# cvxgrp/qcqp

Hardware: AMD Instinct MI355X
Metric: restarts x coord-sweeps / sec (improve COORD_DESCENT phase-2 sweeps, 2n^2 flops each; whole step timed) (higher is better)
Workload: dtype f64

## Files before the change

qcqp_amd/csrc/capi.hip:

```cpp
#include <dlfcn.h>
#include <unistd.h>
#include <hip/hip_runtime.h>
#include <rccl/rccl.h>

#include <algorithm>
#include <cmath>
#include <cstdarg>
#include <cstdio>
#include <cstring>
#include <string>
#include <chrono>
#include <vector>

#include "../../include/qcqp_mi.h"
#include "kernels.hip"
#include "admm.h"
#include "admm_fused.h"
#include "cd_queue.h"
#include "cd_life.h"
#include "gemm_pk.h"
#include "cd_general.h"
#include "cd_dense.h"
#include "sdr_solve.h"

// ... 129 lines not shown
    double stream_limit = 16e9;
    double *dn_gp_pre = nullptr, *dn_tmp = nullptr;
    ncclComm_t comm = nullptr;
    int rank = 0, world = 1;
    double *d_comm = nullptr, *d_comm_big = nullptr;
    int64_t comm_big_cap = 0;
    long long *d_prof = nullptr;
    int cd_stage = 0;
    int64_t Xi_cap = 0;
    bool sdr_factor_resident = false;
    double ad_Minv_rho = 0.0;
    bool ad_Minv_device = false;
    const char *last_cd2_kernel = "";
    bool profile = false;
    int dbg = 0;
    char *af_work = nullptr;
    size_t af_work_cap = 0;
    bool ad_fused = true;
    int ad_fused_nt = 512;
    const char *last_admm_kernel = "";
    int last_admm_C = 0;
    long long af_prof[16] = {0};
    int cd_queue = 2;
    int *d_qnext = nullptr;
    bool q_prepared = false;
    CdLife *d_life = nullptr;
    int Kreal = 0;
    double fbound = 0.0;
    double *l2_scratch = nullptr; size_t l2_scratch_cap = 0;
    double *l2_D = nullptr, *l2_S = nullptr;
    int *l2_abort = nullptr;
    int *l2_cuslot = nullptr;
    double *l2_preslack = nullptr; int64_t l2_preslack_cap = 0;
    double *lr_L = nullptr, *lr_G = nullptr, *lr_U = nullptr; int lr_RB = 0;
    int life_version = 0;
    long long *d_life_prof = nullptr;
    int64_t *d_bestK_idx = nullptr; double *d_bestK_key = nullptr, *d_bestK_x = nullptr; int64_t bestK_cap = 0;
    bool cd_ref_order = false;
    bool force_generic = false;
    std::vector<int> last_st1, last_st2;
};

namespace {

void admm_free(qcqpmi_ctx *c, bool keep_zsolver);

int fail(qcqpmi_ctx *c, int code, const char *fmt, ...) {
    char buf[1024];
    va_list ap;
    va_start(ap, fmt);
    vsnprintf(buf, sizeof(buf), fmt, ap);
    va_end(ap);
    if (c) c->err = buf; else g_create_error = buf;
    return code;
}

#define HIPCHK(c, expr)                                                                       \
    do {                                                                                      \
        hipError_t e_ = (expr);                                                               \
        if (e_ != hipSuccess)                                                                 \
            return fail(c, QCQPMI_EHIP, "%s failed: %s (%s:%d)", #expr, hipGetErrorString(e_), \
                        __FILE__, __LINE__);                                                  \
    } while (0)

template <typename T>
int dev_alloc(qcqpmi_ctx *c, T **p, size_t count, bool zero = true) {
// ... 452 lines not shown
    if (!out || n <= 0 || m < 0) return fail(nullptr, QCQPMI_EINVAL, "ctx_create: bad arguments");
    int ndev = qcqpmi_device_count();
    if (ndev <= 0)
        return fail(nullptr, QCQPMI_EHIP, "no HIP device visible: the qcqp_amd engine requires an MI355X (there is no CPU fallback)");
    if (device < 0 || device >= ndev) return fail(nullptr, QCQPMI_EINVAL, "device %d out of range (%d visible)", device, ndev);
    qcqpmi_ctx *c = new qcqpmi_ctx();
    c->device = device; c->n = n; c->m = m; c->n16 = (n + 15) / 16 * 16;
    c->quads.resize((size_t)m + 1);
    if (const char *sl = getenv("QCQPMI_STREAM_LIMIT")) { const double v = atof(sl); if (v > 0.0) c->stream_limit = v; }
    hipError_t e = hipSetDevice(device);
    if (e == hipSuccess) e = hipStreamCreateWithFlags(&c->stream, hipStreamNonBlocking);
    for (int i = 0; i < 5 && e == hipSuccess; i++) {
        e = hipEventCreate(&c->timers[i].beg);
        if (e == hipSuccess) e = hipEventCreate(&c->timers[i].end);
    }
    if (e != hipSuccess) {
        int rc = fail(nullptr, QCQPMI_EHIP, "ctx_create: %s", hipGetErrorString(e));
        delete c;
        return rc;
    }
    *out = c;
    return 0;
}

void qcqpmi_ctx_destroy(qcqpmi_ctx *c) {
    if (!c) return;
    (void)hipSetDevice(c->device);
    if (c->stream) (void)spin_sync(c->stream);
    if (c->comm && rccl() && rccl()->CommDestroy) rccl()->CommDestroy(c->comm);
    free_population(c);
    admm_free(c, false);
    for (void *p : c->prob_allocs) (void)hipFree(p);
    void *ptrs[] = {c->d_Fpack, c->d_Frow, c->d_mu, c->d_best_idx, c->d_best_key, c->d_comm, c->d_comm_big,
                    c->dn_G, c->dn_Dg, c->dn_Ft, c->dn_prof, c->dn_state, c->d_planes, c->d_out, c->d_wS, c->d_wY, c->d_ww, c->d_wz, c->af_work, c->d_qnext, c->d_life, c->d_life_prof, c->d_bestK_idx, c->d_bestK_key, c->d_bestK_x, c->l2_scratch, c->l2_D, c->l2_S, c->l2_abort, c->l2_cuslot, c->l2_preslack, c->lr_L, c->lr_G, c->lr_U};
    if (c->h_out) (void)hipHostFree(c->h_out);
    if (c->h_pin) (void)hipHostFree(c->h_pin);
    for (void *p : ptrs) if (p) (void)hipFree(p);
    for (auto &t : c->timers) { if (t.beg) (void)hipEventDestroy(t.beg); if (t.end) (void)hipEventDestroy(t.end); }
    for (auto &e : c->dn_ev) if (e) (void)hipEventDestroy(e);
    for (auto &e : c->dn_evn) if (e) (void)hipEventDestroy(e);
    if (c->dn_hn) (void)hipHostFree(c->dn_hn);
    if (c->stream2) (void)hipStreamDestroy(c->stream2);
    if (c->stream) (void)hipStreamDestroy(c->stream);
    delete c;
}

int qcqpmi_set_quad(qcqpmi_ctx *c, int64_t k, int format, const double *vals, const int64_t *idx,
                    const int64_t *ptr, int64_t nnz, const double *q, double r, int relop) {
    if (!c) return QCQPMI_EINVAL;
    if (c->finalized) return fail(c, QCQPMI_ESTATE, "set_quad after finalize");
    if (k < 0 || k > c->m || !q) return fail(c, QCQPMI_EINVAL, "set_quad: bad k or q");
    if ((k == 0) != (relop == 0) || relop < 0 || relop > 2)
        return fail(c, QCQPMI_EINVAL, "set_quad: relop %d invalid for function %lld", relop, (long long)k);
    HostQuad &h = c->quads[(size_t)k];
    h = HostQuad();
    const int64_t n = c->n;
    if (format == QCQPMI_FMT_DENSE) {
        if (!vals) return fail(c, QCQPMI_EINVAL, "set_quad: dense vals missing");
        for (int64_t i = 0; i < n; i++)
            for (int64_t j = 0; j < n; j++) {
                double v = vals[i * n + j];
                if (v != 0.0) { h.ci.push_back((int)i); h.cj.push_back((int)j); h.cv.push_back(v); }
            }
    } else if (format == QCQPMI_FMT_CSR) {
        if (!ptr || (nnz > 0 && (!idx || !vals))) return fail(c, QCQPMI_EINVAL, "set_quad: CSR arrays missing");
        for (int64_t i = 0; i < n; i++)
            for (int64_t e = ptr[i]; e < ptr[i + 1]; e++) {
// ... 737 lines not shown
    const bool lr = use2 && factor_rb > 0 && nmw == 3 && (kind == L2_KIND_BAND || kind == L2_KIND_GEN);
    if (lr) cs2 = 0;
    if (!use2) {
        if (!eligible || c->life_version != 1)
            return fail(c, QCQPMI_EUNSUPPORTED, "cd_stream_run: the lifecycle kernel needs separable constraints -- at most four classes of coordinates, at most two constraints "
                        "per coordinate --, a diagonal of P0 that is positive everywhere or zero everywhere, and 48 <= n <= 2304: use qcqpmi_cd_run per population");
        const int NBq = (int)(c->n16 / 16);
        cs = (c->dbg & 128) ? ((c->dbg >> 8) & 7) : 4;
        cs = cs > RQ_CSMAX ? RQ_CSMAX : cs;
        if (cs >= NBq) cs = 0;
        cs &= ~1;
        if (NBq - cs > RQ_NSIMD * RQ_MAXU || NBq < 3) return fail(c, QCQPMI_EUNSUPPORTED, "cd_stream_run: n = %lld outside the range of cd_phase2_qs_kernel (n <= 1024, at least 3 blocks of 16)", (long long)c->n);
    }
    if (generate && (rc = pop_reserve(c, K * R))) return rc;
    if (!c->d_qnext && (rc = dev_alloc(c, &c->d_qnext, 16))) return rc;
    if (!c->d_life) HIPCHK(c, hipMalloc((void **)&c->d_life, sizeof(CdLife)));
    HIPCHK(c, hipMemsetAsync(c->d_qnext, 0, 16 * sizeof(int), c->stream));
    CdLife L;
    L.on = 1; L.generate = generate ? 1 : 0; L.phase1 = phase1 ? 1 : 0; L.Rtotal = K * R; L.Rpop = R;
    L.seed = seed; L.seed_stride = seed_stride; L.first_index = first_index; L.first_stride = first_stride; L.viol_tol = viol_tol;
    L.sweeps1 = c->d_sweeps1; L.status1 = c->d_status1; L.ran2 = c->d_flag;
    L.prof = nullptr;
    const char *pre_ev = getenv("QCQPMI_L2_PREBUILT");
    const bool pre = lr && !(pre_ev && atoi(pre_ev) == 0);
    L.prebuilt = pre ? 1 : 0; L.preslack = nullptr;
    if (pre) {
        if (K * R > c->l2_preslack_cap) {
            if (c->l2_preslack) { HIPCHK(c, spin_sync(c->stream)); (void)hipFree(c->l2_preslack); c->l2_preslack = nullptr; c->l2_preslack_cap = 0; }
            if ((rc = dev_alloc(c, &c->l2_preslack, (size_t)(K * R)))) return rc;
            c->l2_preslack_cap = K * R;
        }
        L.preslack = c->l2_preslack;
    }
    if (c->profile) {
        if (!c->d_life_prof) HIPCHK(c, hipMalloc((void **)&c->d_life_prof, 24 * sizeof(long long)));
        HIPCHK(c, hipMemsetAsync(c->d_life_prof, 0, 24 * sizeof(long long), c->stream));
        L.prof = c->d_life_prof;
    }
    HIPCHK(c, hipMemcpyAsync(c->d_life, &L, sizeof(L), hipMemcpyHostToDevice, c->stream));
    HIPCHK(c, spin_sync(c->stream));
    int cus = 0;
    HIPCHK(c, hipDeviceGetAttribute(&cus, hipDeviceAttributeMultiprocessorCount, c->device));
    stm[1] = stnow();
    if (use2) {
        if ((rc = cd_life2_reserve(c, nmw, cus))) return rc;
        if (!lr && (c->dbg & 128)) { const int k2 = (c->dbg >> 8) & 7; if (nmw == 3 && (k2 == 0 || k2 == 2 || k2 == 4) && k2 < (int)(c->n16 / 16)) cs2 = k2; }
        const int tiles = cd_life2_tiles(c->dp, nmw, cs2, K * R, cus, 0, lr ? 1 : 0);
        int64_t wgs = (K * R + 16 * tiles - 1) / (16 * tiles);
        const int maxw = cd_life2_max_wgs(nmw, cus, tiles);
        if (wgs > maxw) wgs = maxw;
        if (c->dbg & 1024) { const int lim = (c->dbg >> 12) & 1023; if (lim > 0 && wgs > lim) wgs = lim; }
        CdLife2Args qa;
        qa.P = c->dp; qa.num_iters = num_iters; qa.tol = tol; qa.life = c->d_life;
        cd_queue_fill_batch(c, qa.b, seed, first_index);
        qa.b.R = K * R;
        qa.scratch = c->l2_scratch; qa.Dpack = c->l2_D; qa.Spack = c->l2_S; qa.abort = c->l2_abort; qa.fbound = c->fbound;
        { const char *ev = getenv("QCQPMI_L2_ROT"); const int rot = ev ? atoi(ev) : (lr ? 2 : 0); qa.cuslot = rot ? c->l2_cuslot : nullptr; qa.rotmode = rot; }
        if (qa.cuslot) HIPCHK(c, hipMemsetAsync(c->l2_cuslot, 0, 4096 * sizeof(int), c->stream));
        qa.dbg = (c->dbg & 2048) ? 1 : 0;
        qa.Gpack = lr ? c->lr_G : nullptr; qa.Upack = lr ? c->lr_U : nullptr; qa.RB = lr ? c->lr_RB : 0;
        qa.nclass = c->Kreal;
        const double l0 = stnow();
        (void)hipEventRecord(c->timers[2].beg, c->stream);
        const double l1 = stnow();
        hipError_t qe = pre ? (hipError_t)cd_life2_prep_launch(c->dp, c->d_life, c->X, K * R, num_iters, tol, c->stream) : hipSuccess;
        if (qe == hipSuccess) qe = (hipError_t)cd_life2_launch(qa, nmw, cs2, kind, tiles, (int)wgs, c->stream);
        const double l2 = stnow();
        (void)hipEventRecord(c->timers[2].end, c->stream);
        c->timers[2].valid = true;
        if (qe != hipSuccess) return fail(c, QCQPMI_EHIP, "cd_stream_run: %s", hipGetErrorString(qe));
        c->last_cd2_kernel = cd_life2_name(nmw, kind, tiles, lr ? 1 : 0);
        int ab = 0;
        HIPCHK(c, spin_sync(c->stream));
        const double l3 = stnow();
        HIPCHK(c, hipMemcpyAsync(&ab, c->l2_abort, sizeof(int), hipMemcpyDeviceToHost, c->stream));
        const double l4 = stnow();
        HIPCHK(c, spin_sync(c->stream));
        if (stt) fprintf(stderr, "cd_stream_run launch (ms): reserve %.3f, event %.3f, launch call %.3f, event + spin wait %.3f, copy call %.3f, sync %.3f\n", l0 - stm[1], l1 - l0, l2 - l1, l3 - l2, l4 - l3, stnow() - l4);
        if (ab) {
            HIPCHK(c, hipMemsetAsync(c->l2_abort, 0, sizeof(int), c->stream));
            c->R = 0;
            return fail(c, QCQPMI_EHIP, "cd_stream_run: a wait inside cd_life_kernel ran into its watchdog (internal error; no results)");
        }
    } else {
        CdQueueArgs qa;
        qa.P = c->dp; qa.num_iters = num_iters; qa.tol = tol;
        qa.life = c->d_life; qa.life_on = 1;
        cd_queue_fill_batch(c, qa.b, seed, first_index);
        qa.b.R = K * R;
        (void)hipEventRecord(c->timers[2].beg, c->stream);
        hipError_t qe = (hipError_t)cd_queue_launch(qa, cs, cus, c->stream);
        (void)hipEventRecord(c->timers[2].end, c->stream);
        c->timers[2].valid = true;
        if (qe != hipSuccess) return fail(c, QCQPMI_EHIP, "cd_stream_run: %s", hipGetErrorString(qe));
        HIPCHK(c, spin_sync(c->stream));
        c->last_cd2_kernel = "cd_phase2_qs_kernel<lifecycle>";
    }
    c->cd_stage = 0;
// ... 318 lines not shown
```

qcqp_amd/csrc/capi_admm.inc:

```

namespace {

struct RocblasApi {
    void *h = nullptr;
    int (*create)(void **) = nullptr;
    int (*destroy)(void *) = nullptr;
    int (*set_stream)(void *, hipStream_t) = nullptr;
};

RocblasApi *rocblas() {
    static RocblasApi api;
    static bool tried = false;
    if (!tried) {
        tried = true;
        const char *names[] = {"librocblas.so", "librocblas.so.5", "/opt/rocm/lib/librocblas.so"};
        for (const char *nm : names) {
            api.h = dlopen(nm, RTLD_NOW | RTLD_GLOBAL);
            if (api.h) break;
        }
        if (api.h) {
            api.create = (decltype(api.create))dlsym(api.h, "rocblas_create_handle");
            api.destroy = (decltype(api.destroy))dlsym(api.h, "rocblas_destroy_handle");
            api.set_stream = (decltype(api.set_stream))dlsym(api.h, "rocblas_set_stream");
        }
// ... 464 lines not shown
    const int64_t idx = (int64_t)blockIdx.x * blockDim.x + threadIdx.x;
    if (idx >= n16 * n16) return;
    const int64_t t = idx / (n16 * 16), rem = idx % (n16 * 16), i = rem / 16, j = 16 * t + (rem & 15);
    Xtm[idx] = (i == j) ? alpha : 0.0;
}

__global__ void zs_pack_sym_kernel(const double *__restrict__ Xtm, double *__restrict__ Apk, int64_t n16) {
    const int64_t idx = (int64_t)blockIdx.x * blockDim.x + threadIdx.x;
    if (idx >= n16 * n16) return;
    const int l = (int)(idx & 63);
    const int64_t fk = idx >> 6, KS = n16 / 4, rb = fk / KS, kk = fk % KS;
    Apk[idx] = Xtm[rb * n16 * 16 + (4 * kk + (l >> 4)) * 16 + (l & 15)];
}

__global__ void zs_update_kernel(double *__restrict__ Xtm, const double *__restrict__ Utm, const double *__restrict__ Ttm,
                                 int64_t n16, unsigned long long *__restrict__ resid_bits) {
    const int64_t idx = (int64_t)blockIdx.x * blockDim.x + threadIdx.x;
    double r = 0.0;
    if (idx < n16 * n16) {
        const int64_t t = idx / (n16 * 16), rem = idx % (n16 * 16), i = rem / 16, j = 16 * t + (rem & 15);
        Xtm[idx] = 2.0 * Xtm[idx] - Utm[idx];
        r = fabs(Ttm[idx] - (i == j ? 1.0 : 0.0));
    }
    __shared__ double red[256];
    red[threadIdx.x] = r;
    __syncthreads();
    for (int s = 128; s > 0; s >>= 1) {
        if ((int)threadIdx.x < s) red[threadIdx.x] = fmax(red[threadIdx.x], red[threadIdx.x + s]);
        __syncthreads();
    }
    if (threadIdx.x == 0) atomicMax(resid_bits, (unsigned long long)__double_as_longlong(red[0]));
}

int qcqpmi_admm_zsolver_device(qcqpmi_ctx *c, double rho, int64_t max_iter, double *resid_out, int64_t *iters_out) {
    if (!c) return QCQPMI_EINVAL;
    if (!c->finalized) return fail(c, QCQPMI_ESTATE, "admm_zsolver_device: context not finalized");
    HIPCHK(c, hipSetDevice(c->device));
    const int64_t n = c->n, n16 = c->n16, m = c->m, tot = n16 * n16;
    const int KBn = (int)(n16 / 16), nt = KBn;
    if (max_iter <= 0) max_iter = 80;
    hipStream_t st = c->stream;
    int rc;
    DevBuf<double> Mtm, Mpk, Xtm, Xpk, Ttm, Utm, rs;
    DevBuf<unsigned long long> rb;
    if ((rc = dev_alloc(c, &Mtm.p, (size_t)tot, false)) || (rc = dev_alloc(c, &Mpk.p, (size_t)tot, false)) ||
        (rc = dev_alloc(c, &Xtm.p, (size_t)tot, false)) || (rc = dev_alloc(c, &Xpk.p, (size_t)tot, false)) ||
        (rc = dev_alloc(c, &Ttm.p, (size_t)tot, false)) || (rc = dev_alloc(c, &Utm.p, (size_t)tot, false)) ||
        (rc = dev_alloc(c, &rs.p, (size_t)n16, false)) || (rc = dev_alloc(c, &rb.p, 1, false)))
        return rc;
    const dim3 gb((unsigned)((tot + 255) / 256)), tb(256);
    hipLaunchKernelGGL(zs_build_kernel, gb, tb, 0, st, c->dp.P0, n, n16, rho * (double)m, Mtm.p);
    hipLaunchKernelGGL(zs_pack_sym_kernel, gb, tb, 0, st, (const double *)Mtm.p, Mpk.p, n16);
    hipLaunchKernelGGL(zs_rowsum_kernel, dim3((unsigned)((n16 + 255) / 256)), tb, 0, st, (const double *)Mtm.p, n16, rs.p);
    HIPCHK(c, hipGetLastError());
    std::vector<double> hrs((size_t)n16);
    HIPCHK(c, hipMemcpyAsync(hrs.data(), rs.p, (size_t)n16 * sizeof(double), hipMemcpyDeviceToHost, st));
    HIPCHK(c, spin_sync(st));
    double nrm = 0.0;
    for (double v : hrs) nrm = std::max(nrm, v);
    if (!(nrm > 0.0) || !std::isfinite(nrm)) return fail(c, QCQPMI_EINVAL, "admm_zsolver_device: 2 (P0 + rho m I) is zero or not finite");
    hipLaunchKernelGGL(zs_scaled_identity_kernel, gb, tb, 0, st, Xtm.p, n16, 1.0 / nrm);
    double resid = INFINITY, prev = INFINITY;
    int64_t it = 0;
    for (; it < max_iter; it++) {
        hipLaunchKernelGGL(zs_pack_sym_kernel, gb, tb, 0, st, (const double *)Xtm.p, Xpk.p, n16);
        if ((rc = gemm_pk(c, Mpk.p, Xtm.p, Ttm.p, nullptr, KBn, KBn, nt, 1))) return rc;
        if ((rc = gemm_pk(c, Xpk.p, Ttm.p, Utm.p, nullptr, KBn, KBn, nt, 1))) return rc;
        HIPCHK(c, hipMemsetAsync(rb.p, 0, sizeof(unsigned long long), st));
        hipLaunchKernelGGL(zs_update_kernel, gb, tb, 0, st, Xtm.p, (const double *)Utm.p, (const double *)Ttm.p, n16, rb.p);
        HIPCHK(c, hipGetLastError());
        unsigned long long bits = 0;
        HIPCHK(c, hipMemcpyAsync(&bits, rb.p, sizeof bits, hipMemcpyDeviceToHost, st));
        HIPCHK(c, spin_sync(st));
        double r;
        memcpy(&r, &bits, sizeof r);
        prev = resid; resid = r;
        if (!std::isfinite(resid)) return fail(c, QCQPMI_EREFERENCE, "admm_zsolver_device: iteration diverged (is P0 + rho m I positive definite?)");
        if (resid < 1e-7 && (resid * resid < 1e-15 || resid >= 0.5 * prev)) { it++; break; }
        if (it > 8 && resid > 1.0 - 1e-12 && prev > 1.0 - 1e-12 && resid >= prev)
            return fail(c, QCQPMI_EREFERENCE, "admm_zsolver_device: no contraction (is P0 + rho m I positive definite?)");
    }
    if (!(resid < 1e-7)) return fail(c, QCQPMI_EREFERENCE, "admm_zsolver_device: not converged after %lld iterations (residual %.3e)", (long long)it, resid);
    if (c->ad_Minvpk) { (void)hipFree(c->ad_Minvpk); c->ad_Minvpk = nullptr; }
    if ((rc = dev_alloc(c, &c->ad_Minvpk, (size_t)tot, false))) return rc;
    hipLaunchKernelGGL(zs_pack_sym_kernel, gb, tb, 0, st, (const double *)Xtm.p, c->ad_Minvpk, n16);
    HIPCHK(c, hipGetLastError());
    HIPCHK(c, spin_sync(st));
    c->ad_Minv_rho = rho;
    c->ad_Minv_device = true;
    if (resid_out) *resid_out = resid * resid;
    if (iters_out) *iters_out = it;
    return 0;
}

__global__ __launch_bounds__(256) void p0_gemv_kernel(const double *__restrict__ P0, const double *__restrict__ v, int64_t n, int64_t n16,
                                                      double *__restrict__ y) {
    const int lane = threadIdx.x & 63;
    const int64_t row = (int64_t)blockIdx.x * 4 + (threadIdx.x >> 6);
    if (row >= n) return;
    const double *pr = P0 + row * n16;
    double s = 0.0;
    for (int64_t j = lane; j < n; j += 64) s += pr[j] * v[j];
    for (int off = 32; off > 0; off >>= 1) s += __shfl_down(s, off, 64);
    if (lane == 0) y[row] = s;
}

static double tridiag_min_eig(const std::vector<double> &al, const std::vector<double> &be, int k) {
    double lo = INFINITY, hi = -INFINITY;
    for (int i = 0; i < k; i++) {
        const double r = (i > 0 ? fabs(be[i - 1]) : 0.0) + (i + 1 < k ? fabs(be[i]) : 0.0);
        lo = std::min(lo, al[i] - r); hi = std::max(hi, al[i] + r);
    }
    auto count_below = [&](double x) {
        int cnt = 0; double d = 1.0;
        for (int i = 0; i < k; i++) {
// ... 466 lines not shown
```

qcqp_amd/csrc/cd_life.h:

```cpp
#pragma once
#include <hip/hip_runtime.h>
#include <stdint.h>
#include "kernels.h"
#include "cd_queue.h"

namespace qcqpmi {

enum { L2_KIND_BAND = 0, L2_KIND_GEN = 1, L2_KIND_LIN = 2, L2_KIND_GENK = 3, L2_KIND_LINK = 4 };

struct CdLife2Args {
    DevProblem P;
    CdBatch b;
    int64_t num_iters;
    double tol;
    const CdLife *life;
    double *scratch;
    const double *Dpack;
    const double *Spack;
    int *abort;
    int *cuslot;
    double fbound;
    const double *Gpack, *Upack;
    int RB;
    int rotmode;
    int nclass;
    int dbg;
};

bool cd_life2_config(const DevProblem &P, int Kreal, int objclass, bool symcls, int factor_rb, int *nmw, int *cs, int *kind);
size_t cd_life2_lds_bytes(int nmw, int cs, int tiles, int lr, int kind);
bool cd_life2_factor_ok(const DevProblem &P, int64_t r);
int cd_life2_pack_factor(const double *Lrow, double *Gpack, double *Upack, int NB, int RB, hipStream_t st);
int cd_life2_max_wgs(int nmw, int cus, int tiles);
int cd_life2_tiles(const DevProblem &P, int nmw, int cs, int64_t restarts, int cus, int requested, int lr);
int cd_life2_pack(const DevProblem &P, double *Dpack, double *Spack, hipStream_t st);
int cd_life2_prep_launch(const DevProblem &P, const CdLife *life, double *X, int64_t Rtotal, int64_t num_iters, double tol, hipStream_t st);
int cd_life2_launch(const CdLife2Args &a, int nmw, int cs, int kind, int tiles, int wgs, hipStream_t st);
const char *cd_life2_name(int nmw, int kind, int tiles, int lr);

}
```

qcqp_amd/csrc/cd_life.hip:

```cpp
#include "cd_life.h"

#include <cstdio>
#include <cstdlib>

#include "onevar.h"
#include "cd_phase1_sep.h"

namespace qcqpmi {
typedef double v4d __attribute__((ext_vector_type(4)));
template <typename XPtr>
__device__ inline v4d block_rows_times_X(const double *__restrict__ Ab, XPtr Xs, int kk0, int kk1, int lane, v4d acc) {
    const int xoff = (lane >> 4) * 16 + (lane & 15);
    for (int kk = kk0; kk < kk1; kk++) acc = __builtin_amdgcn_mfma_f64_16x16x4f64(Ab[(int64_t)kk * 64 + lane], Xs[kk * 64 + xoff], acc, 0, 0, 0);
    return acc;
}
}

#include "cd_phase2_q.h"

namespace qcqpmi {
namespace {

#define LG __attribute__((address_space(1)))
template <class T>
// ... 1184 lines not shown
                const int st = tid >> 4, sc = tid & 15;
                double mvx;
                if (lf_pre) {
                    const int id = l2_tl(sid, st, TD)[sc];
                    mvx = l2_g(lf->preslack)[id];
                    l2_tl(p1sw, st, TD)[sc] = (int)l2_g(lf->sweeps1)[id];
                    l2_tl(p1st, st, TD)[sc] = l2_g(lf->status1)[id];
                    l2_tl(gatep, st, TD)[sc] = l2_g(lf->ran2)[id];
                } else {
                    mvx = l2_unkey(l2_tl(p1key, st, TD)[sc]);
                    l2_tl(gatep, st, TD)[sc] = (mvx < lf_viol_tol && l2_tl(p1st, st, TD)[sc] == 0) ? 1 : 0;
                }
                l2_tl(slk, st, TD)[sc] = mvx;
                L2_STORE_SETS(st, sc, mvx)
            }
            __syncthreads();
            if (nlast < 16) {
                for (int w = tid; w < NS * (16 - nlast); w += NT) {
                    const int c = w % NS, ct = c >> 4, cc = c & 15, row = w / NS;
                    if (l2_tl(snew, ct, TD)[cc] || l2_tl(sid, ct, TD)[cc] < 0) {
                        const int nn = l2_tl(TC.n, ct, TD)[cc];
                        double xp = 0.0;
                        if (BK == L2_KIND_BAND) xp = nn >= 2 ? l2_tl(TC.lo, ct, TD)[16 * KCLV + cc] : 0.0;
                        else if (BK == L2_KIND_GEN) xp = nn >= 1 ? l2_tl(TC.hi, ct, TD)[cc] : 0.0;
                        else xp = nn >= 2 ? l2_tl(TC.hi, ct, TD)[16 * KCLV + cc] : l2_tl(TC.hi, ct, TD)[cc];
                        if (!(xp == xp) || __builtin_isinf(xp)) xp = 0.0;
                        (Xg0 + (int64_t)ct * n16 * 16)[(P.n + row) * 16 + cc] = xp;
                    }
                }
                __syncthreads();
            }
            if (LR) {
                const int r16 = 16 * a0.RB;
                for (int w = tid; w < NS * (32 + r16); w += NT) {
                    const int c = w % NS, ct = c >> 4, cc = c & 15, rowz = w / NS;
                    if (l2_tl(snew, ct, TD)[cc] || l2_tl(sid, ct, TD)[cc] < 0) {
                        if (rowz < 32) l2_tl(pend, ct, TD)[rowz * 16 + cc] = 0.0;
                        else l2_tl(ytile, ct, TD)[(rowz - 32) * 16 + cc] = 0.0;
                    }
                }
                __syncthreads();
            }
            if (lf->prof && tid == 0) {
                int nn = 0;
                for (int k = 0; k < NS; k++) nn += l2_tl(snew, k >> 4, TD)[k & 15] ? 1 : 0;
                atomicAdd((unsigned long long *)lf->prof + 0, (unsigned long long)((long long)__builtin_amdgcn_s_memtime() - pt0));
                atomicAdd((unsigned long long *)lf->prof + 2, 1ull);
                atomicAdd((unsigned long long *)lf->prof + 3, (unsigned long long)nn);
            }
            __builtin_amdgcn_s_setprio(0);
        }
        if (role == 0) {
            long long *cs_ = l2_tl(cst, rtile, TD);
            if (l2_tl(snew, rtile, TD)[r]) {
#pragma unroll
                for (int f = 0; f < 6; f++) cs_[f * 64 + lane] = 0;
                const int pass = l2_tl(gatep, rtile, TD)[r];
                cs_[6 * 64 + lane] = 0;
                cs_[4 * 64 + lane] = (pass && !PRE && !LR) ? 0 : 1;
                cs_[7 * 64 + lane] = (pass ? (PRE ? 4 : 0) : 1) | (LR ? 8 : 0);
                cs_[8 * 64 + lane] = 0;
            } else if (l2_tl(sid, rtile, TD)[r] < 0) {
                cs_[4 * 64 + lane] = 1; cs_[6 * 64 + lane] = 0;
                cs_[7 * 64 + lane] = 2; cs_[8 * 64 + lane] = 0;
            }
        }
        __syncthreads();
        if (tid == 0 && l2_g(lifep)->prof) *(long long *)(ctl + 6) = (long long)__builtin_amdgcn_s_memtime();

        if (role > 0) {
            if (LR) l2_mfma_lr_role<NMW>(role - 1, rtile);
            else l2_mfma_role<NMW, CS>(role - 1, rtile);
        } else l2_chain_role<NMW, CS, KIND, TILES, LR>(rtile);

        __syncthreads();
        if (sy[L2_ABORT] || (TILES > 1 && l2_tl((int *)sy, 1, TD)[L2_ABORT])) {
            if (tid == 0) __hip_atomic_store(l2_g(a0.abort), 1, __ATOMIC_RELAXED, __HIP_MEMORY_SCOPE_AGENT);
            break;
        }
        if (tid == 0 && l2_g(lifep)->prof)
        {
            const long long now_ = (long long)__builtin_amdgcn_s_memtime();
            atomicAdd((unsigned long long *)l2_g(lifep)->prof + 5, (unsigned long long)(now_ - *(long long *)(ctl + 6)));
            atomicAdd((unsigned long long *)l2_g(lifep)->prof + 20, (unsigned long long)(now_ - *(long long *)(ctl + 8)));
        }
        {
            const int e0 = P.cptr[P.krep[0]];
            const double cp = P.cp[e0], cq = P.cq[e0], cr = P.cr[e0];
            const int rel = P.crel[e0];
            if (tid == 0) { int cnt = 0; for (int k = 0; k < NS; k++) if (l2_tl(sfin, k >> 4, TD)[k & 15]) p1cols[cnt++] = k; ctl[4] = cnt; }
            if (tid < NS) l2_tl(p1key, tid >> 4, TD)[tid & 15] = l2_key(-QM_INF);
            __syncthreads();
            const int nfin = ctl[4];
// ... 27 lines not shown
                                const double vv = (rel == RELOP_EQ) ? fabs(f) : (f > 0.0 ? f : 0.0);
                                atomicMax(&l2_tl(p1key, col >> 4, TD)[col & 15], l2_key(vv));
                            }
                        }
                    }
                }
            }
            __syncthreads();
            if (tid < NS && l2_tl(sfin, tid >> 4, TD)[tid & 15]) {
                const int st = tid >> 4, sc = tid & 15;
                const double mx = l2_unkey(l2_tl(p1key, st, TD)[sc]);
                const int id = l2_tl(sid, st, TD)[sc];
                l2_g(a0.b.visits)[id] = l2_tl(ovis, st, TD)[sc]; l2_g(a0.b.accepted)[id] = l2_tl(oacc, st, TD)[sc]; l2_g(a0.b.sweeps)[id] = l2_tl(oswp, st, TD)[sc];
                l2_g(a0.b.status)[id] = l2_tl(ost, st, TD)[sc];
                if (a0.b.f0out) l2_g(a0.b.f0out)[id] = l2_tl(of0, st, TD)[sc];
                if (a0.b.mvout) l2_g(a0.b.mvout)[id] = mx;
                LG const CdLife *lf = l2_g(lifep);
                l2_g(lf->sweeps1)[id] = l2_tl(p1sw, st, TD)[sc]; l2_g(lf->status1)[id] = l2_tl(p1st, st, TD)[sc];
                l2_g(lf->ran2)[id] = (uint8_t)l2_tl(gatep, st, TD)[sc];
                l2_tl(sid, st, TD)[sc] = -1; l2_tl(sfin, st, TD)[sc] = 0;
            }
            __syncthreads();
        }
    }
    if (tid0 == 0 && lf0->prof) {
        const unsigned long long dtl = (unsigned long long)((long long)__builtin_amdgcn_s_memtime() - life_t0);
        atomicAdd((unsigned long long *)lf0->prof + 1, dtl);
        atomicMax((unsigned long long *)lf0->prof + 16, dtl);
    }
}

#undef L2_STORE_SETS

constexpr int L2P_NT = 256;
__global__ __launch_bounds__(L2P_NT) void cd_life_prep_kernel(DevProblem P, const CdLife *life, double *X, int64_t num_iters, double tol) {
    __shared__ unsigned long long key[16];
    __shared__ int upd[16], st1[16], fin[16], sw[16], nact;
    const int tid = threadIdx.x, s = tid & 15, g = tid >> 4;
    LG const CdLife *lf = l2_g(life);
    const int64_t id = (int64_t)blockIdx.x * 16 + s;
    const bool valid = id < lf->Rtotal;
    const int64_t n = P.n, n16 = P.n16;
    LG double *Xt = l2_g(X) + (int64_t)blockIdx.x * n16 * 16 + s;
    const double viol_tol = lf->viol_tol;
    uint64_t sd = 0, gidx = 0;
    if (valid) {
        const uint64_t pop = (uint64_t)id / (uint64_t)lf->Rpop, rho = (uint64_t)id % (uint64_t)lf->Rpop;
        sd = lf->seed + pop * lf->seed_stride;
        gidx = lf->first_index + pop * lf->first_stride + rho;
    }
    if (lf->generate && valid) {
        for (int64_t j = 2 * g; j < n16; j += 32) {
            double xo = 0.0;
            const double xe = (j < n) ? l2_keyed_normal_pair(sd, gidx, (uint64_t)j, &xo) : 0.0;
            Xt[16 * j] = xe;
            Xt[16 * (j + 1)] = (j + 1 < n) ? xo : 0.0;
        }
    }
    const int e0 = P.cptr[P.krep[0]];
    const double cp = P.cp[e0], cq = P.cq[e0], cr = P.cr[e0];
    const int rel = P.crel[e0];
    if (tid < 16) { fin[tid] = valid ? 0 : 1; sw[tid] = 0; st1[tid] = 0; }
    if (lf->phase1) {
        const bool band2 = cq == 0.0 && rel == RELOP_EQ && cp > 1e-4 && cr < -1e-3;
        for (int64_t t = 0; t < num_iters; t++) {
            if (tid < 16) { key[tid] = l2_key(-QM_INF); upd[tid] = 0; }
            __syncthreads();
            if (tid == 0) { int c = 0; for (int k = 0; k < 16; k++) c += fin[k] ? 0 : 1; nact = c; }
// ... 36 lines not shown
            }
            if ((tid & 63) < 16 && !fin[s]) { atomicMax(&key[s], l2_key(va)); if (moved) upd[s] = 1; }
            if (stv) st1[s] = stv;
            __syncthreads();
            if (tid < 16 && !fin[tid]) {
                sw[tid]++;
                if (l2_unkey(key[tid]) < viol_tol || !upd[tid]) fin[tid] = 1;
            }
        }
    }
    __syncthreads();
    if (tid < 16) key[tid] = l2_key(-QM_INF);
    __syncthreads();
    double v = -QM_INF;
    if (valid)
        for (int64_t j = 2 * g; j < n; j += 32)
            for (int64_t i = j; i < j + 2 && i < n; i++) {
                const double x = Xt[16 * i];
                const double f = (cp * x + cq) * x + cr;
                const double w = (rel == RELOP_EQ) ? fabs(f) : (f > 0.0 ? f : 0.0);
                v = w > v ? w : v;
            }
#pragma unroll
    for (int o = 16; o <= 32; o <<= 1) { const double w = __shfl_xor(v, o, 64); v = w > v ? w : v; }
    if ((tid & 63) < 16 && valid) atomicMax(&key[s], l2_key(v));
    __syncthreads();
    if (tid < 16 && valid) {
        const double mvx = l2_unkey(key[tid]);
        l2_g(const_cast<double *>(lf->preslack))[id] = mvx;
        l2_g(lf->sweeps1)[id] = sw[tid];
        l2_g(lf->status1)[id] = st1[tid];
        l2_g(lf->ran2)[id] = (mvx < viol_tol && st1[tid] == 0) ? 1 : 0;
    }
}

__global__ void l2_pack_kernel(DevProblem P, double *Dpack, double *Spack) {
    const int b = blockIdx.x, t = threadIdx.x;
    const int64_t n16 = P.n16;
    const int rr = t >> 4, cc = t & 15;
    Dpack[(int64_t)b * 256 + t] = (cc > rr) ? P.P0[(16 * (int64_t)b + rr) * n16 + 16 * b + cc] : 0.0;
    if (t < 16) {
        const int64_t i = 16 * (int64_t)b + t;
        const double d = P.P0[i * n16 + i], rc = P.rcp2d[i];
        Spack[(int64_t)b * 48 + t] = 0.5 * P.q0[i];
        Spack[(int64_t)b * 48 + 16 + t] = rc + rc;
        Spack[(int64_t)b * 48 + 32 + t] = d;
    }
}

__global__ void l2_pack_factor_kernel(const double *__restrict__ L, double *__restrict__ Gpack, double *__restrict__ Upack, int NB, int RB) {
    const int64_t idx = (int64_t)blockIdx.x * blockDim.x + threadIdx.x;
    if (idx >= (int64_t)NB * RB * 256) return;
    const int e = (int)(idx & 1), lane = (int)((idx >> 1) & 63), vp = (int)((idx >> 7) & 1);
    const int64_t rest = idx >> 8;
    const int beta = (int)(rest % RB), b = (int)(rest / RB), v = 2 * vp + e;
    const int64_t r16 = 16 * (int64_t)RB;
    Gpack[idx] = L[(16 * (int64_t)b + (lane & 15)) * r16 + 16 * beta + 4 * v + (lane >> 4)];
    Upack[idx] = L[(16 * (int64_t)b + 4 * v + (lane >> 4)) * r16 + 16 * beta + (lane & 15)];
}

template <int NMW, int CS, int TILES, int LR>
int l2_launch_kind(const CdLife2Args &a, int kind, int wgs, size_t lds, hipStream_t st) {
    constexpr bool MK = TILES == 1 && !LR;
    if (!MK && (kind == L2_KIND_GENK || kind == L2_KIND_LINK)) return (int)hipErrorInvalidValue;
    auto k = kind == L2_KIND_BAND ? cd_life_kernel<NMW, CS, L2_KIND_BAND, TILES, LR> : (kind == L2_KIND_GEN || LR) ? cd_life_kernel<NMW, CS, L2_KIND_GEN, TILES, LR>
             : kind == L2_KIND_GENK ? cd_life_kernel<NMW, CS, MK ? L2_KIND_GENK : L2_KIND_GEN, TILES, LR>
             : kind == L2_KIND_LINK ? cd_life_kernel<NMW, CS, MK ? L2_KIND_LINK : L2_KIND_GEN, TILES, LR>
                                    : cd_life_kernel<NMW, CS, LR ? L2_KIND_GEN : L2_KIND_LIN, TILES, LR>;
    hipError_t e = hipFuncSetAttribute((const void *)k, hipFuncAttributeMaxDynamicSharedMemorySize, (int)lds);
    if (e != hipSuccess) return (int)e;
    hipLaunchKernelGGL(k, dim3((unsigned)wgs), dim3((NMW == 3 && TILES == 1) ? 256 : 512), lds, st, a);
    return (int)hipGetLastError();
}

}

size_t cd_life2_lds_bytes(int nmw, int cs, int tiles, int lr, int kind) {
    const bool multi = kind == L2_KIND_GENK || kind == L2_KIND_LINK;
    return ((size_t)L2_SHARED_DOUBLES + (size_t)tiles * (size_t)l2_tile_doubles(nmw, cs > 0 ? cs : 1, lr, multi ? L2_KCL : 1, multi ? 2 : 1)) * sizeof(double) + 256;
}

bool cd_life2_factor_ok(const DevProblem &P, int64_t r) {
    const int64_t r16 = (r + 15) / 16 * 16;
    if (r < 1 || r16 > 16 * L2_YBMAX || P.NB < 8) return false;
    return true;
}

int cd_life2_pack_factor(const double *Lrow, double *Gpack, double *Upack, int NB, int RB, hipStream_t st) {
    const int64_t tot = (int64_t)NB * RB * 256;
    hipLaunchKernelGGL(l2_pack_factor_kernel, dim3((unsigned)((tot + 255) / 256)), dim3(256), 0, st, Lrow, Gpack, Upack, NB, RB);
    return (int)hipGetLastError();
}

int cd_life2_prep_launch(const DevProblem &P, const CdLife *life, double *X, int64_t Rtotal, int64_t num_iters, double tol, hipStream_t st) {
    hipLaunchKernelGGL(cd_life_prep_kernel, dim3((unsigned)((Rtotal + 15) / 16)), dim3(L2P_NT), 0, st, P, life, X, num_iters, tol);
    return (int)hipGetLastError();
}

int cd_life2_max_wgs(int nmw, int cus, int tiles) { return (nmw == 3 && tiles == 1) ? 2 * cus : cus; }

bool cd_life2_config(const DevProblem &P, int Kreal, int objclass, bool symcls, int factor_rb, int *nmw, int *cs, int *kind) {
    if (!P.sep || P.maxc < 1 || P.maxc > 2 || Kreal < 1 || Kreal > L2_KCL) return false;
    const bool multi = P.maxc > 1 || Kreal > 1;
    if (objclass != 1 && objclass != 2) return false;
    const int NB = (int)P.NB;
    if (NB < 3) return false;
    int w, c;
    if (NB <= 4) { w = 3; c = 0; }
    else if (NB - 4 <= 3 * RQ_MAXU) { w = 3; c = (NB < 8) ? 2 : 4; }
    else if (factor_rb > 0 && !multi && objclass == 1 && NB <= 256) { w = 3; c = 0; }
    else if (NB - 4 <= 7 * RQ_MAXU) { w = 7; c = 4; }
    else return false;
    *nmw = w; *cs = c;
    *kind = multi ? (objclass == 2 ? L2_KIND_LINK : L2_KIND_GENK) : objclass == 2 ? L2_KIND_LIN : (symcls ? L2_KIND_BAND : L2_KIND_GEN);
    return true;
}

int cd_life2_tiles(const DevProblem &P, int nmw, int cs, int64_t restarts, int cus, int requested, int lr) {
    (void)P; (void)restarts; (void)cus;
    if (!lr || nmw != 3 || cs != 0) return 1;
    int t = requested;
    if (const char *ev = getenv("QCQPMI_L2_TILES")) t = atoi(ev);
    return t == 2 ? 2 : 1;
}

int cd_life2_pack(const DevProblem &P, double *Dpack, double *Spack, hipStream_t st) {
    hipLaunchKernelGGL(l2_pack_kernel, dim3((unsigned)P.NB), dim3(256), 0, st, P, Dpack, Spack);
    return (int)hipGetLastError();
// ... 45 lines not shown
```

qcqp_amd/csrc/cd_queue.h:

```cpp
#pragma once
#include <hip/hip_runtime.h>
#include <stdint.h>
#include "kernels.h"

namespace qcqpmi {

struct CdBatch {
    double *X;
    const double *f0cur;
    const double *slack;
    const uint8_t *flag;
    int64_t *visits, *accepted, *sweeps;
    int *status;
    double *f0out, *mvout;
    int64_t R;
    uint64_t seed, first_index;
    int *next;
};

struct CdLife {
    int on;
    int generate;
    int phase1;
    int64_t Rtotal, Rpop;
    uint64_t seed, seed_stride, first_index, first_stride;
    double viol_tol;
    int64_t *sweeps1;
    int *status1;
    uint8_t *ran2;
    long long *prof;
    int prebuilt;
    const double *preslack;
};

struct CdQueueArgs {
    DevProblem P;
    CdBatch b;
    int64_t num_iters;
    double tol;
    const CdLife *life;
    int life_on;
};

size_t cd_queue_lds_bytes(const DevProblem &P);
int cd_queue_launch(const CdQueueArgs &a, int cs, int max_wgs, hipStream_t st);

}
```

Before: 28.13 million.

## Precompute low-rank Y0 projections in prep kernel with MFMA and preload into tiles

In the prebuilt low-rank CD path, the prep kernel now also computes each restart's initial low-rank projection Y0 = U^T x with f64 MFMA and writes it to a new device buffer. The main life kernel then copies these precomputed values into its tiles for newly started restarts, instead of zeroing them and rebuilding them in-kernel. This moves per-restart setup work out of the latency-bound CD kernel into a parallel prep pass, at the cost of extra memory traffic and a buffer of up to 2 GB. Separately, the ADMM z-solver gains a refinement step (a compensated-dot residual, a GEMM and an add) that improves the accuracy of the computed inverse.

```diff
diff --git a/qcqp_amd/csrc/capi.hip b/qcqp_amd/csrc/capi.hip
--- a/qcqp_amd/csrc/capi.hip
+++ b/qcqp_amd/csrc/capi.hip
@@ -185,6 +185,7 @@
     int *l2_abort = nullptr;
     int *l2_cuslot = nullptr;
     double *l2_preslack = nullptr; int64_t l2_preslack_cap = 0;
+    double *l2_y0 = nullptr; size_t l2_y0_cap = 0;
     double *lr_L = nullptr, *lr_G = nullptr, *lr_U = nullptr; int lr_RB = 0;
     int life_version = 0;
     long long *d_life_prof = nullptr;
@@ -703,7 +704,7 @@
     admm_free(c, false);
     for (void *p : c->prob_allocs) (void)hipFree(p);
     void *ptrs[] = {c->d_Fpack, c->d_Frow, c->d_mu, c->d_best_idx, c->d_best_key, c->d_comm, c->d_comm_big,
-                    c->dn_G, c->dn_Dg, c->dn_Ft, c->dn_prof, c->dn_state, c->d_planes, c->d_out, c->d_wS, c->d_wY, c->d_ww, c->d_wz, c->af_work, c->d_qnext, c->d_life, c->d_life_prof, c->d_bestK_idx, c->d_bestK_key, c->d_bestK_x, c->l2_scratch, c->l2_D, c->l2_S, c->l2_abort, c->l2_cuslot, c->l2_preslack, c->lr_L, c->lr_G, c->lr_U};
+                    c->dn_G, c->dn_Dg, c->dn_Ft, c->dn_prof, c->dn_state, c->d_planes, c->d_out, c->d_wS, c->d_wY, c->d_ww, c->d_wz, c->af_work, c->d_qnext, c->d_life, c->d_life_prof, c->d_bestK_idx, c->d_bestK_key, c->d_bestK_x, c->l2_scratch, c->l2_D, c->l2_S, c->l2_abort, c->l2_cuslot, c->l2_preslack, c->l2_y0, c->lr_L, c->lr_G, c->lr_U};
     if (c->h_out) (void)hipHostFree(c->h_out);
     if (c->h_pin) (void)hipHostFree(c->h_pin);
     for (void *p : ptrs) if (p) (void)hipFree(p);
@@ -1507,6 +1508,24 @@
         }
         L.preslack = c->l2_preslack;
     }
+    L.y0 = nullptr;
+    const char *y0_ev = getenv("QCQPMI_L2_Y0");
+    if (pre && !(y0_ev && atoi(y0_ev) == 0)) {
+        const size_t need = (size_t)((K * R + 15) / 16) * 16 * 16 * (size_t)c->lr_RB;
+        const char *bud_ev = getenv("QCQPMI_L2_Y0_BUDGET_MB");
+        const size_t budget = bud_ev ? (size_t)std::max(0LL, atoll(bud_ev)) << 20 : (size_t)2 << 30;
+        if (need * sizeof(double) <= budget) {
+            if (need > c->l2_y0_cap) {
+                if (c->l2_y0) { HIPCHK(c, spin_sync(c->stream)); (void)hipFree(c->l2_y0); c->l2_y0 = nullptr; c->l2_y0_cap = 0; }
+                size_t fr = 0, tot = 0;
+                if (hipMemGetInfo(&fr, &tot) == hipSuccess && need * sizeof(double) <= fr / 2) {
+                    if ((rc = dev_alloc(c, &c->l2_y0, need, false))) return rc;
+                    c->l2_y0_cap = need;
+                }
+            }
+            if (need <= c->l2_y0_cap) L.y0 = c->l2_y0;
+        }
+    }
     if (c->profile) {
         if (!c->d_life_prof) HIPCHK(c, hipMalloc((void **)&c->d_life_prof, 24 * sizeof(long long)));
         HIPCHK(c, hipMemsetAsync(c->d_life_prof, 0, 24 * sizeof(long long), c->stream));
@@ -1538,7 +1557,7 @@
         const double l0 = stnow();
         (void)hipEventRecord(c->timers[2].beg, c->stream);
         const double l1 = stnow();
-        hipError_t qe = pre ? (hipError_t)cd_life2_prep_launch(c->dp, c->d_life, c->X, K * R, num_iters, tol, c->stream) : hipSuccess;
+        hipError_t qe = pre ? (hipError_t)cd_life2_prep_launch(c->dp, c->d_life, c->X, K * R, num_iters, tol, c->lr_U, c->lr_RB, c->stream) : hipSuccess;
         if (qe == hipSuccess) qe = (hipError_t)cd_life2_launch(qa, nmw, cs2, kind, tiles, (int)wgs, c->stream);
         const double l2 = stnow();
         (void)hipEventRecord(c->timers[2].end, c->stream);
diff --git a/qcqp_amd/csrc/capi_admm.inc b/qcqp_amd/csrc/capi_admm.inc
--- a/qcqp_amd/csrc/capi_admm.inc
+++ b/qcqp_amd/csrc/capi_admm.inc
@@ -520,6 +520,26 @@
     if (threadIdx.x == 0) atomicMax(resid_bits, (unsigned long long)__double_as_longlong(red[0]));
 }
 
+__global__ void zs_resid_dot2_kernel(const double *__restrict__ Mtm, const double *__restrict__ Xtm, int64_t n16, double *__restrict__ Rtm) {
+    const int64_t idx = (int64_t)blockIdx.x * blockDim.x + threadIdx.x;
+    if (idx >= n16 * n16) return;
+    const int64_t t = idx / (n16 * 16), rem = idx % (n16 * 16), i = rem / 16, j = 16 * t + (rem & 15);
+    double s = (i == j) ? 1.0 : 0.0, cmp = 0.0;
+    for (int64_t k = 0; k < n16; k++) {
+        const double a = -Mtm[(k / 16) * n16 * 16 + i * 16 + (k & 15)], b = Xtm[t * n16 * 16 + k * 16 + (j & 15)];
+        const double p = a * b, pe = __builtin_fma(a, b, -p);
+        const double sn = s + p, z = sn - s, se = (s - (sn - z)) + (p - z);
+        s = sn;
+        cmp += pe + se;
+    }
+    Rtm[idx] = s + cmp;
+}
+
+__global__ void zs_add_kernel(double *__restrict__ Xtm, const double *__restrict__ Utm, int64_t tot) {
+    const int64_t idx = (int64_t)blockIdx.x * blockDim.x + threadIdx.x;
+    if (idx < tot) Xtm[idx] += Utm[idx];
+}
+
 int qcqpmi_admm_zsolver_device(qcqpmi_ctx *c, double rho, int64_t max_iter, double *resid_out, int64_t *iters_out) {
     if (!c) return QCQPMI_EINVAL;
     if (!c->finalized) return fail(c, QCQPMI_ESTATE, "admm_zsolver_device: context not finalized");
@@ -569,6 +589,12 @@
             return fail(c, QCQPMI_EREFERENCE, "admm_zsolver_device: no contraction (is P0 + rho m I positive definite?)");
     }
     if (!(resid < 1e-7)) return fail(c, QCQPMI_EREFERENCE, "admm_zsolver_device: not converged after %lld iterations (residual %.3e)", (long long)it, resid);
+    hipLaunchKernelGGL(zs_resid_dot2_kernel, gb, tb, 0, st, (const double *)Mtm.p, (const double *)Xtm.p, n16, Ttm.p);
+    hipLaunchKernelGGL(zs_pack_sym_kernel, gb, tb, 0, st, (const double *)Xtm.p, Xpk.p, n16);
+    HIPCHK(c, hipGetLastError());
+    if ((rc = gemm_pk(c, Xpk.p, Ttm.p, Utm.p, nullptr, KBn, KBn, nt, 1))) return rc;
+    hipLaunchKernelGGL(zs_add_kernel, gb, tb, 0, st, Xtm.p, (const double *)Utm.p, tot);
+    HIPCHK(c, hipGetLastError());
     if (c->ad_Minvpk) { (void)hipFree(c->ad_Minvpk); c->ad_Minvpk = nullptr; }
     if ((rc = dev_alloc(c, &c->ad_Minvpk, (size_t)tot, false))) return rc;
     hipLaunchKernelGGL(zs_pack_sym_kernel, gb, tb, 0, st, (const double *)Xtm.p, c->ad_Minvpk, n16);
diff --git a/qcqp_amd/csrc/cd_life.h b/qcqp_amd/csrc/cd_life.h
--- a/qcqp_amd/csrc/cd_life.h
+++ b/qcqp_amd/csrc/cd_life.h
@@ -34,7 +34,8 @@
 int cd_life2_max_wgs(int nmw, int cus, int tiles);
 int cd_life2_tiles(const DevProblem &P, int nmw, int cs, int64_t restarts, int cus, int requested, int lr);
 int cd_life2_pack(const DevProblem &P, double *Dpack, double *Spack, hipStream_t st);
-int cd_life2_prep_launch(const DevProblem &P, const CdLife *life, double *X, int64_t Rtotal, int64_t num_iters, double tol, hipStream_t st);
+int cd_life2_prep_launch(const DevProblem &P, const CdLife *life, double *X, int64_t Rtotal, int64_t num_iters, double tol, const double *Upack,
+                         int RB, hipStream_t st);
 int cd_life2_launch(const CdLife2Args &a, int nmw, int cs, int kind, int tiles, int wgs, hipStream_t st);
 const char *cd_life2_name(int nmw, int kind, int tiles, int lr);
 
diff --git a/qcqp_amd/csrc/cd_life.hip b/qcqp_amd/csrc/cd_life.hip
--- a/qcqp_amd/csrc/cd_life.hip
+++ b/qcqp_amd/csrc/cd_life.hip
@@ -1240,11 +1240,35 @@
             }
             if (LR) {
                 const int r16 = 16 * a0.RB;
+                LG const double *y0g = l2_g(lf->y0);
                 for (int w = tid; w < NS * (32 + r16); w += NT) {
                     const int c = w % NS, ct = c >> 4, cc = c & 15, rowz = w / NS;
-                    if (l2_tl(snew, ct, TD)[cc] || l2_tl(sid, ct, TD)[cc] < 0) {
+                    if ((l2_tl(snew, ct, TD)[cc] && !y0g) || l2_tl(sid, ct, TD)[cc] < 0) {
                         if (rowz < 32) l2_tl(pend, ct, TD)[rowz * 16 + cc] = 0.0;
                         else l2_tl(ytile, ct, TD)[(rowz - 32) * 16 + cc] = 0.0;
+                    }
+                }
+                if (y0g) {
+                    if (tid == 0) { int cnt = 0; for (int k = 0; k < NS; k++) if (l2_tl(snew, k >> 4, TD)[k & 15]) p1cols[cnt++] = k; ctl[4] = cnt; }
+                    __syncthreads();
+                    const int ry = 32 + r16, items = ctl[4] * ry;
+                    for (int w0 = tid; w0 < items; w0 += 8 * NT) {
+                        double v8[8];
+#pragma unroll
+                        for (int u = 0; u < 8; u++) {
+                            const int w = w0 + u * NT, c = p1cols[w < items ? w / ry : 0], ct = c >> 4, cc = c & 15, row = w % ry;
+                            const int id = l2_tl(sid, ct, TD)[cc];
+                            v8[u] = (w >= items) ? 0.0 : (row < 32) ? (Xg0 + (int64_t)ct * n16 * 16)[(n16 - 32 + row) * 16 + cc]
+                                                                    : y0g[(int64_t)id * r16 + row - 32];
+                        }
+#pragma unroll
+                        for (int u = 0; u < 8; u++) {
+                            const int w = w0 + u * NT, c = p1cols[w < items ? w / ry : 0], ct = c >> 4, cc = c & 15, row = w % ry;
+                            if (w < items) {
+                                if (row < 32) l2_tl(pend, ct, TD)[row * 16 + cc] = v8[u];
+                                else l2_tl(ytile, ct, TD)[(row - 32) * 16 + cc] = v8[u];
+                            }
+                        }
                     }
                 }
                 __syncthreads();
@@ -1264,9 +1288,10 @@
 #pragma unroll
                 for (int f = 0; f < 6; f++) cs_[f * 64 + lane] = 0;
                 const int pass = l2_tl(gatep, rtile, TD)[r];
+                const bool load = LR && l2_g(lifep)->y0 == nullptr;
                 cs_[6 * 64 + lane] = 0;
-                cs_[4 * 64 + lane] = (pass && !PRE && !LR) ? 0 : 1;
-                cs_[7 * 64 + lane] = (pass ? (PRE ? 4 : 0) : 1) | (LR ? 8 : 0);
+                cs_[4 * 64 + lane] = (pass && !PRE && !load) ? 0 : 1;
+                cs_[7 * 64 + lane] = (pass ? (PRE ? 4 : 0) : 1) | (load ? 8 : 0);
                 cs_[8 * 64 + lane] = 0;
             } else if (l2_tl(sid, rtile, TD)[r] < 0) {
                 cs_[4 * 64 + lane] = 1; cs_[6 * 64 + lane] = 0;
@@ -1360,8 +1385,72 @@
 
 #undef L2_STORE_SETS
 
+constexpr int L2Y_U = (L2_YBMAX + 3) / 4;
+template <int T>
+__device__ __attribute__((always_inline)) inline void l2_y0_tiles(const double *X, const double *Upack, double *Y0, int64_t t0, int nt, int64_t n16,
+                                                                  int NB, int RB) {
+    const int lane = threadIdx.x & 63, w = __builtin_amdgcn_readfirstlane(threadIdx.x >> 6);
+    const int nu = (RB > w) ? (RB - w + 3) / 4 : 0;
+    LG const v2d_ *up = (LG const v2d_ *)l2_g(Upack);
+    LG const double *xb[T];
+#pragma unroll
+    for (int t = 0; t < T; t++) xb[t] = l2_g(X) + ((t0 + (t < nt ? t : 0)) * n16 + (lane >> 4)) * 16 + (lane & 15);
+    v4d_ y[L2Y_U][T];
+#pragma unroll
+    for (int u = 0; u < L2Y_U; u++)
+#pragma unroll
+        for (int t = 0; t < T; t++) y[u][t] = v4d_{0.0, 0.0, 0.0, 0.0};
+    v2d_ aU[L2Y_U][2];
+    double bd[T][4];
+    auto load = [&](int b) {
+#pragma unroll
+        for (int u = 0; u < L2Y_U; u++)
+            if (u < nu) {
+                LG const v2d_ *p = up + ((int64_t)b * RB + w + 4 * u) * 128 + lane;
+                aU[u][0] = p[0];
+                aU[u][1] = p[64];
+            }
+#pragma unroll
+        for (int t = 0; t < T; t++)
+#pragma unroll
+            for (int v = 0; v < 4; v++) bd[t][v] = xb[t][(16 * (int64_t)b + 4 * v) * 16];
+    };
+    load(0);
+    for (int b = 0; b <= NB - 3; b++) {
+        v2d_ cU[L2Y_U][2];
+        double cd[T][4];
+#pragma unroll
+        for (int u = 0; u < L2Y_U; u++) { cU[u][0] = aU[u][0]; cU[u][1] = aU[u][1]; }
+#pragma unroll
+        for (int t = 0; t < T; t++)
+#pragma unroll
+            for (int v = 0; v < 4; v++) cd[t][v] = bd[t][v];
+        if (b < NB - 3) load(b + 1);
+#pragma unroll
+        for (int v = 0; v < 4; v++)
+#pragma unroll
+            for (int u = 0; u < L2Y_U; u++)
+                if (u < nu)
+#pragma unroll
+                    for (int t = 0; t < T; t++) y[u][t] = __builtin_amdgcn_mfma_f64_16x16x4f64(cU[u][v >> 1][v & 1], cd[t][v], y[u][t], 0, 0, 0);
+    }
+    const int64_t r16 = 16 * (int64_t)RB;
+#pragma unroll
+    for (int t = 0; t < T; t++)
+        if (t < nt) {
+            LG double *yo = l2_g(Y0) + ((t0 + t) * 16 + (lane & 15)) * r16 + (lane >> 4);
+#pragma unroll
+            for (int u = 0; u < L2Y_U; u++)
+                if (u < nu) {
+#pragma unroll
+                    for (int v = 0; v < 4; v++) yo[16 * (w + 4 * u) + 4 * v] = y[u][t][v];
+                }
+        }
+}
+
 constexpr int L2P_NT = 256;
-__global__ __launch_bounds__(L2P_NT) void cd_life_prep_kernel(DevProblem P, const CdLife *life, double *X, int64_t num_iters, double tol) {
+__global__ __launch_bounds__(L2P_NT, 3) void cd_life_prep_kernel(DevProblem P, const CdLife *life, double *X, int64_t num_iters, double tol,
+                                                              const double *Upack, int RB) {
     __shared__ unsigned long long key[16];
     __shared__ int upd[16], st1[16], fin[16], sw[16], nact;
     const int tid = threadIdx.x, s = tid & 15, g = tid >> 4;
@@ -1464,6 +1553,11 @@
         l2_g(lf->status1)[id] = st1[tid];
         l2_g(lf->ran2)[id] = (mvx < viol_tol && st1[tid] == 0) ? 1 : 0;
     }
+    LG const double *y0 = l2_g(lf->y0);
+    if (y0) {
+        __syncthreads();
+        l2_y0_tiles<1>(X, Upack, const_cast<double *>((const double *)y0), (int64_t)blockIdx.x, 1, n16, (int)(n16 / 16), RB);
+    }
 }
 
 __global__ void l2_pack_kernel(DevProblem P, double *Dpack, double *Spack) {
@@ -1524,8 +1618,10 @@
     return (int)hipGetLastError();
 }
 
-int cd_life2_prep_launch(const DevProblem &P, const CdLife *life, double *X, int64_t Rtotal, int64_t num_iters, double tol, hipStream_t st) {
-    hipLaunchKernelGGL(cd_life_prep_kernel, dim3((unsigned)((Rtotal + 15) / 16)), dim3(L2P_NT), 0, st, P, life, X, num_iters, tol);
+int cd_life2_prep_launch(const DevProblem &P, const CdLife *life, double *X, int64_t Rtotal, int64_t num_iters, double tol, const double *Upack,
+                         int RB, hipStream_t st) {
+    if (RB < 0 || RB > L2_YBMAX || (RB > 0 && !Upack)) return (int)hipErrorInvalidValue;
+    hipLaunchKernelGGL(cd_life_prep_kernel, dim3((unsigned)((Rtotal + 15) / 16)), dim3(L2P_NT), 0, st, P, life, X, num_iters, tol, Upack, RB);
     return (int)hipGetLastError();
 }
 
diff --git a/qcqp_amd/csrc/cd_queue.h b/qcqp_amd/csrc/cd_queue.h
--- a/qcqp_amd/csrc/cd_queue.h
+++ b/qcqp_amd/csrc/cd_queue.h
@@ -31,6 +31,7 @@
     long long *prof;
     int prebuilt;
     const double *preslack;
+    const double *y0;
 };
 
 struct CdQueueArgs {
```

Result: no change. 28.09 million (median of 6 runs) (-0.1%).
